# LouisRouss/DiffuLab

Hardware: AMD Instinct MI355X
Metric: train images/sec/node (DiT-S/2 flow-matching, 256x256 latents) (higher is better)
Workload: dtype bf16

## Files before the change

diffulab_amd/csrc/block.hip:

```cpp
#include <stdlib.h>

#include "common.h"

static thread_local hipEvent_t g_blk_event = nullptr;
static int fork_to_side(hipStream_t main, hipStream_t side) {
  if (main == side) return 0;
  if (!g_blk_event && hipEventCreateWithFlags(&g_blk_event, hipEventDisableTiming) != hipSuccess) return -1;
  if (hipEventRecord(g_blk_event, main) != hipSuccess) return -1;
  return hipStreamWaitEvent(side, g_blk_event, 0) == hipSuccess ? 0 : -1;
}

extern "C" int dl_stream_wait_stream(dl_stream_t waiter, dl_stream_t waited) {
  if (fork_to_side((hipStream_t)waited, (hipStream_t)waiter) != 0) {
    dl_set_error("dl_stream_wait_stream: %s", hipGetErrorString(hipGetLastError()));
    return DL_ERR_LAUNCH;
  }
  return DL_OK;
}
extern "C" int dl_memset_zero(void* p, int64_t bytes, dl_stream_t stream) {
  DL_CHECK_ARG(p && bytes >= 0, "dl_memset_zero: bad args");
  if (bytes && hipMemsetAsync(p, 0, (size_t)bytes, (hipStream_t)stream) != hipSuccess) {
    dl_set_error("dl_memset_zero: %s", hipGetErrorString(hipGetLastError()));
    return DL_ERR_LAUNCH;
  }
// ... 77 lines not shown
  if (rc == DL_ERR_UNSUPPORTED) {
    DL_CHECK_ARG(P(U), "dl_dit_block_fwd: this shape has no fused MLP-up kernel and needs the U buffer");
    RUN(dl_gemm_nt(P(XM2), D, P(W_UP), b->ldw_d, P(U), 2 * F, M, 2 * F, D, nullptr, DL_ACT_NONE, DL_BF16, nullptr, nullptr, 0, nullptr, 0, 1,
                   stream));
    RUN(dl_swiglu_fwd(P(U), P(H), M, F, stream));
  } else if (rc != DL_OK) {
    return rc;
  }
  RUN(dl_gemm_nt(P(H), F, P(W_DOWN), b->ldw_f, P(T2), D, M, D, F, nullptr, DL_ACT_NONE, DL_BF16, nullptr, nullptr, 0, nullptr, 0, 1, stream));
  return DL_OK;
}

extern "C" int dl_dit_block_bwd(const dl_dit_block_t* b, dl_stream_t main_, dl_stream_t side_, int side_wgs) {
  DL_CHECK_ARG(b, "dl_dit_block_bwd: null block");
  hipStream_t main = (hipStream_t)main_, side = (hipStream_t)side_;
  const DlWgCapScope cap_scope(b->max_workgroups);
  const int64_t B = b->B, N = b->N, D = b->D, H = b->H, F = b->F, M = B * N, dh = D / H;
  const float sm = 0.125f;
  dl_wgrad_t wg[4];
  int nwg = 0;
  bool grouped = P(TN_SLAB) != nullptr && ((D % 384 == 0 && F % 192 == 0) || (D % 256 == 0 && F % 256 == 0)) && M % 32 == 0 && M >= 2048;
  auto wgrad = [&](const void* dy, int64_t ldy, const void* x, int64_t ldx, void* g, int64_t Mo, int64_t No) -> int {
    if (grouped) {
      wg[nwg++] = dl_wgrad_t{dy, ldy, x, ldx, (float*)g, Mo, No};
      return DL_OK;
    }
    if (fork_to_side(main, side)) return DL_ERR_LAUNCH;
    return dl_gemm_tn_ex(dy, ldy, x, ldx, (float*)g, No, Mo, No, M, side_wgs, side);
  };
  auto fold = [&](void* partial, void* g) -> int {
    if (fork_to_side(main, side)) return DL_ERR_LAUNCH;
    return dl_reduce_rows_f32((float*)partial, (float*)g, B, 2 * D, 1, side);
  };
  RUN(wgrad(P(DT2), D, P(H), F, P(G_DOWN), D, F));
  if (P(U)) {
    RUN(dl_gemm_nt(P(DT2), D, P(WT_DOWN), b->ldwt_d, P(DH), F, M, F, D, nullptr, DL_ACT_NONE, DL_BF16, nullptr, nullptr, 0, nullptr, 0, 1, main));
    RUN(dl_swiglu_bwd(P(DH), P(U), P(DU), M, F, main));
  } else {
    RUN(dl_mlp_dswiglu_recompute(P(XM2), D, P(W_UP_PERM), b->ldw_d, P(DT2), D, P(WT_DOWN), b->ldwt_d, P(DU), 2 * F, M, F, D, D, main));
  }
  RUN(wgrad(P(DU), 2 * F, P(XM2), D, P(G_UP), 2 * F, D));
  const bool rows = (b->row_gemms & 1) != 0, fold_here = (b->row_gemms & 4) == 0;
  if (rows) {
    RUN(dl_ln_modulate_gemm_bwd(P(DU), 2 * F, P(WT_UP), b->ldwt_f2, M, 2 * F, P(X1), (const float*)P(LN2_W), (const float*)P(LN2_B),
                                P(SCALE2), b->ld_mod, N, (const float*)P(MEAN2), (const float*)P(RSTD2), P(DX_IN), P(DX_MID),
                                (float*)P(DSCALE2), (float*)P(DSHIFT2), b->ld_dmod, (float*)P(DWB2), P(T1), P(GATE1), b->ld_mod, P(DT1),
                                (float*)P(DGATE1), D, main));
  } else {
    RUN(dl_gemm_nt(P(DU), 2 * F, P(WT_UP), b->ldwt_f2, P(DXM), D, M, D, 2 * F, nullptr, DL_ACT_NONE, DL_BF16, nullptr, nullptr, 0, nullptr,
                   0, 1, main));
    RUN(dl_ln_modulate_bwd(P(DXM), P(X1), (const float*)P(LN2_W), (const float*)P(LN2_B), P(SCALE2), b->ld_mod, N,
                           (const float*)P(MEAN2), (const float*)P(RSTD2), P(DX_IN), P(DX_MID), (float*)P(DSCALE2), (float*)P(DSHIFT2),
                           b->ld_dmod, (float*)P(DWB2), P(T1), P(GATE1), b->ld_mod, P(DT1), (float*)P(DGATE1), M, D, main));
  }
  if (fold_here) RUN(fold(P(DWB2), P(G_LN2)));
  RUN(wgrad(P(DT1), D, P(A), D, P(G_PROJ), D, D));
  RUN(dl_gemm_nt(P(DT1), D, P(WT_PROJ), b->ldwt_d, P(DA), D, M, D, D, nullptr, DL_ACT_NONE, DL_BF16, nullptr, nullptr, 0, nullptr, 0, 1, main));
  const bool v_in_place = P(V) == nullptr;
  if (v_in_place && P(QK_PARTIALS) && D <= 512) {
    RUN(dl_attn_bwd_tok(P(Q), P(K), P(QKV), P(A), P(DA), (const float*)P(LSE), P(DQKV), B, H, N, dh, sm, main));
    RUN(dl_qk_norm_rope_bwd_inplace(P(QKV), (const float*)P(QN_SCALE), (const float*)P(KN_SCALE), (const float*)P(ROPE_COS),
                                    (const float*)P(ROPE_SIN), (const float*)P(RRMS), P(DQKV), (float*)P(G_QK_SCALE),
                                    (float*)P(QK_PARTIALS), B, N, H, dh, b->rot, nullptr, main));
  } else {
    if (v_in_place)
      RUN(dl_attn_bwd_sv(P(Q), P(K), (const char*)P(QKV) + 2 * D * 2, N * 3 * D, dh, 3 * D, P(A), P(DA), (const float*)P(LSE), P(DQ), P(DK),
// ... 31 lines not shown
```

diffulab_amd/csrc/block_fused.hip:

```cpp
#include <stdlib.h>

#include "common.h"
#include "attention_body.h"
#include "gemm_rows_body.h"
#include "gemm_stationary_body.h"

#define CH_THREADS 512
#define CH_NKS 6

struct ChainRowGemm {
  const bf16_t* A;
  int64_t lda;
  const bf16_t* W;
  int64_t ldw;
  int K;
  RowEpi ep;
};
struct ChainAttn {
  const bf16_t* qkv;
  bf16_t* out;
  float* lse;
  int H;
  float scale;
  QkNorm qn;
};
struct ChainArgs {
  int B;
  StArgs qkv;
  ChainAttn attn;
  ChainRowGemm proj;
  StArgs up;
  ChainRowGemm down;
};

constexpr int ch_max(int a, int b) { return a > b ? a : b; }
constexpr int ch_lds_bytes() { return ch_max(ch_max(st_lds_bytes<CH_NKS>(), 2 * RK_STAGE), attn_pipe_lds_bytes(RK_BN)); }

static __device__ __forceinline__ void ch_phase_sync() {
  asm volatile("s_waitcnt vmcnt(0) lgkmcnt(0)" ::: "memory");
  __builtin_amdgcn_fence(__ATOMIC_RELEASE, "workgroup");
  __syncthreads();
  __builtin_amdgcn_fence(__ATOMIC_ACQUIRE, "workgroup");
}

static __device__ __forceinline__ const ChainArgs* ch_args() {
  auto p = __builtin_amdgcn_kernarg_segment_ptr();
  asm volatile("" : "+s"(p));
  return (const ChainArgs*)p;
}
static __device__ __forceinline__ int ch_tid() {
  int t = threadIdx.x;
  asm volatile("" : "+v"(t));
  return t;
}
static __device__ __forceinline__ void ch_row_gemm(const ChainRowGemm* gp, char* smem, int sample) {
  const ChainRowGemm g = *gp;
  rk_gemm_body<RK_LNF>(g.A, g.lda, g.W, g.ldw, RK_BN, g.K, g.ep, smem, ch_tid(), sample, 0, 1);
}
template <int EPI>
static __device__ __forceinline__ void ch_st_gemm(const StArgs* ap, char* smem, int sample) {
  const StArgs a = *ap;
  st_gemm_body<CH_NKS, EPI>(a, smem, ch_tid(), sample, 0, 1);
}
static __device__ __forceinline__ void ch_attention(const ChainAttn* ap, char* smem, int sample) {
  const ChainAttn a = *ap;
  attn_qkn_pipe_body(a.qkv, a.out, a.lse, a.H, a.scale, a.qn, smem, ch_tid(), sample * a.H, 1, a.H);
}

__global__ __launch_bounds__(CH_THREADS, 2) void dit_block_fwd_chain_k(ChainArgs a) {
  extern __shared__ __attribute__((aligned(16))) char smem[];
  for (int s = blockIdx.x; s < a.B; s += gridDim.x) {
    ch_st_gemm<1>(&ch_args()->qkv, smem, s);
    ch_phase_sync();
    ch_attention(&ch_args()->attn, smem, s);
    ch_phase_sync();
    ch_row_gemm(&ch_args()->proj, smem, s);
    ch_phase_sync();
    ch_st_gemm<0>(&ch_args()->up, smem, s);
    ch_phase_sync();
    ch_row_gemm(&ch_args()->down, smem, s);
    ch_phase_sync();
  }
}

#define P(k) (b->p[DL_BLK_##k])
#define CH_ALIGNED16(p) ((((uintptr_t)(p)) & 15) == 0)

static void ch_row_epi(RowEpi& ep, const void* resid, const void* gate, int64_t ld_gate, const void* ln_w, const void* ln_b,
                       const void* scale, const void* shift, int64_t ld_mod, float eps, void* t_out, void* x_out, void* xm_out,
                       void* mean, void* rstd) {
// ... 59 lines not shown
                     (const float*)P(ROPE_SIN), (bf16_t*)(train ? P(Q) : nullptr), (bf16_t*)(train ? P(K) : nullptr),
                     (float*)(train ? P(RRMS) : nullptr), 1.0f / (float)D, 1e-6f, (int)b->rot, (int)(3 * D)};
  a.proj.A = (const bf16_t*)P(A);
  a.proj.lda = D;
  a.proj.W = (const bf16_t*)P(W_PROJ);
  a.proj.ldw = b->ldw_d;
  a.proj.K = (int)D;
  ch_row_epi(a.proj.ep, P(X_IN), P(GATE1), b->ld_mod, P(LN2_W), P(LN2_B), P(SCALE2), P(SHIFT2), b->ld_mod, b->eps, P(T1), P(X1), P(XM2),
             P(MEAN2), P(RSTD2));
  a.up = StArgs{(const bf16_t*)P(XM2), D, (const bf16_t*)P(W_UP_PERM), b->ldw_d, (bf16_t*)u, 2 * F, (bf16_t*)P(H), F, (int)F, nullptr, 0,
                (int)(B * N), (int)(2 * F)};
  a.down.A = (const bf16_t*)P(H);
  a.down.lda = F;
  a.down.W = (const bf16_t*)P(W_DOWN);
  a.down.ldw = b->ldw_f;
  a.down.K = (int)F;
  ch_row_epi(a.down.ep, P(X1), P(GATE2), b->ld_mod, P(NEXT_LN_W), P(NEXT_LN_B), P(NEXT_SCALE), P(NEXT_SHIFT), b->ld_mod, b->next_eps,
             P(T2), P(NEXT_X), P(NEXT_XM), P(NEXT_MEAN), P(NEXT_RSTD));

  constexpr int LDS = ch_lds_bytes();
  static_assert(LDS <= 160 * 1024, "the chain kernel's LDS is the largest phase's");
  static DevOnce once;
  const int n_cu = dev_cus(once, [] {
    (void)hipFuncSetAttribute((const void*)dit_block_fwd_chain_k, hipFuncAttributeMaxDynamicSharedMemorySize, LDS);
  });
  const DlWgCapScope cap_scope(b->max_workgroups);
  const int budget = dl_wg_budget(n_cu);
  int grid = (int)(B < budget ? B : budget);
  if (b->max_workgroups > 0 && b->max_workgroups < grid) grid = b->max_workgroups;
  hipLaunchKernelGGL(dit_block_fwd_chain_k, grid, CH_THREADS, LDS, (hipStream_t)stream, a);
  DL_LAUNCH_CHECK();
  return DL_OK;
}
```

diffulab_amd/csrc/gemm_stationary_body.h:

```cpp
#ifndef DIFFULAB_GEMM_STATIONARY_BODY_H
#define DIFFULAB_GEMM_STATIONARY_BODY_H

#include <type_traits>

#include "common.h"

#define ST_THREADS 512
#define ST_PANEL 256
#define ST_ROWS 64

typedef __attribute__((address_space(3))) void st_lds_void_t;
typedef const __attribute__((address_space(1))) void st_glb_void_t;

struct StArgs {
  const bf16_t* X;
  int64_t ldx;
  const bf16_t* W;
  int64_t ldw;
  bf16_t* C;
  int64_t ldc;
  bf16_t* H;
  int64_t ldh;
  int F;
  float* ssq;
// ... 96 lines not shown
          auto sh = __builtin_amdgcn_permlane32_swap(__float_as_uint(hv[e]), __float_as_uint(hv[4 + e]), false, false);
          v1[e] = __uint_as_float(s1[0]);
          v1[4 + e] = __uint_as_float(s1[1]);
          v3[e] = __uint_as_float(s3[0]);
          v3[4 + e] = __uint_as_float(s3[1]);
          h8[e] = __uint_as_float(sh[0]);
          h8[4 + e] = __uint_as_float(sh[1]);
        }
#pragma unroll
        for (int e = 0; e < 16; ++e) c[e] = 0.f;
        if (a.C) {
          *(u32x4_t*)(a.C + (int64_t)m * a.ldc + u0) = pack8(v1);
          *(u32x4_t*)(a.C + (int64_t)m * a.ldc + a.F + u0) = pack8(v3);
        }
        *(u32x4_t*)(a.H + (int64_t)m * a.ldh + u0) = pack8(h8);
      }
    } else {
#pragma unroll
      for (int j = 0; j < 2; ++j)
#pragma unroll
        for (int gp = 0; gp < 2; ++gp) {
          f32x16_t& c = acc[2 * HALF + j];
          float v[8];
#pragma unroll
          for (int e = 0; e < 4; ++e) {
            auto sw2 = __builtin_amdgcn_permlane32_swap(__float_as_uint(c[8 * gp + e]), __float_as_uint(c[8 * gp + 4 + e]), false, false);
            v[e] = __uint_as_float(sw2[0]);
            v[4 + e] = __uint_as_float(sw2[1]);
            c[8 * gp + e] = 0.f;
            c[8 * gp + 4 + e] = 0.f;
          }
          const u32x4_t pk = pack8(v);
          *(u32x4_t*)(a.C + (int64_t)m * a.ldc + n_base + j * 32 + 16 * gp + 8 * hi) = pk;
          float r[8];
          unpack8(pk, r);
#pragma unroll
          for (int e = 0; e < 8; ++e) ss += r[e] * r[e];
        }
      if (st % 6 == 2) {
        ss_lo = xor32_sum(ss);
        ss = 0.f;
      }
      if ((st + 1) % 6 == 0 || st + 1 == S) {
        if (st / 6 < a.ssq_tiles) {
          const float t = ss_lo + xor32_sum(ss);
          if (hi == 0) a.ssq[(int64_t)m * a.ssq_tiles + st / 6] = t;
        }
        ss = 0.f;
        ss_lo = 0.f;
      }
    }
  };

  int it = 0;
  auto stage = [&](auto half_tag, int st) {
    constexpr int HALF = decltype(half_tag)::value;
    constexpr int YOUNG = (NST - 2) * NKS;
    if (it + NST - 2 < total) {
      if (st < 2) st_wait_vmcnt<YOUNG>();
      else if (EPI == 1) st_wait_vmcnt<YOUNG + 4>();
      else if (a.C) st_wait_vmcnt<YOUNG + 6>();
      else st_wait_vmcnt<YOUNG + 2>();
    } else {
      st_wait_vmcnt<0>();
    }
    __builtin_amdgcn_s_barrier();
    if (NST < 3 && s_it < total) stage_next();
    if (upper && st > 0) epilogue(std::integral_constant<int, 1 - HALF>{}, st - 1);
    const unsigned sw = smem_lds + (it % NST) * STAGE + rd_base;
    bf16x8_t wq[PD + 1];
    auto rd = [&](int s) {
      const int f = s >> 1;
      const unsigned ad = sw + (((f & 7) << 5) ^ rd_x);
      bf16x8_t& v = wq[s % (PD + 1)];
      switch ((f >> 3) * 2 + (s & 1)) {
        case 0: st_lds_read<0>(v, ad); break;
        case 1: st_lds_read<32 * PITCH>(v, ad); break;
        case 2: st_lds_read<256>(v, ad); break;
        case 3: st_lds_read<32 * PITCH + 256>(v, ad); break;
        case 4: st_lds_read<512>(v, ad); break;
        case 5: st_lds_read<32 * PITCH + 512>(v, ad); break;
        case 6: st_lds_read<768>(v, ad); break;
        default: st_lds_read<32 * PITCH + 768>(v, ad); break;
      }
    };
#pragma unroll
    for (int s = 0; s < PD; ++s) rd(s);
#pragma unroll
    for (int s = 0; s < 2 * NF; ++s) {
      __builtin_amdgcn_sched_barrier(0);
      if (s + PD < 2 * NF) rd(s + PD);
      st_lds_landed_n(2 * NF - 1 - s < PD ? 2 * NF - 1 - s : PD, wq[s % (PD + 1)]);
      acc[2 * HALF + (s & 1)] =
// ... 29 lines not shown
```

diffulab_amd/engine.py:

```python

from __future__ import annotations

import functools
import math
from dataclasses import dataclass, field

import torch
from torch import Tensor

from . import ops, tuning


_PARAM_EPOCH = 0


def bump_param_epoch() -> None:
    global _PARAM_EPOCH
    _PARAM_EPOCH += 1


def _must(ok: bool) -> None:
    if not ok:
        raise RuntimeError("a HIP kernel declined a shape the engine had selected it for")

# ... 584 lines not shown
        blk.ldwt_3d = sh[pre + "attention.qkv.weight|t"].stride(0)
        blk.rot, blk.eps = sum(d.rope_axes_dim), 1e-5
        blk.max_workgroups = self._main_wgs()
        prev = None
        if i > 0:
            ap = w["layers"][(i - 1) if train else 0]
            prev = (ap["x1"], ap["t2"], mrow((i - 1) * 6 * D + 5 * D))
        blk.set(x_in=xin, pend_x=prev[0] if prev else None, pend_t=prev[1] if prev else None, pend_gate=prev[2] if prev else None,
                scale1=mrow(mo), shift1=mrow(mo + D), gate1=mrow(mo + 2 * D), scale2=mrow(mo + 3 * D), shift2=mrow(mo + 4 * D),
                gate2=mrow(mo + 5 * D),
                ln1_w=self.P(pre + "norm_1.weight"), ln1_b=self.P(pre + "norm_1.bias"), ln2_w=self.P(pre + "norm_2.weight"),
                ln2_b=self.P(pre + "norm_2.bias"), qn_scale=self.P(pre + "attention.qk_norm.query_norm.scale"),
                kn_scale=self.P(pre + "attention.qk_norm.key_norm.scale"),
                w_qkv=sh[pre + "attention.qkv.weight|f"], w_proj=sh[pre + "attention.proj_out.weight|f"],
                w_up=sh[pre + "mlp_input.0.weight|f"], w_up_perm=sh[pre + "mlp_input.0.weight|g"], w_down=sh[pre + "mlp_input.2.weight|f"],
                wt_qkv=sh[pre + "attention.qkv.weight|t"], wt_proj=sh[pre + "attention.proj_out.weight|t"],
                wt_up=sh[pre + "mlp_input.0.weight|t"], wt_down=sh[pre + "mlp_input.2.weight|t"], rope_cos=cos, rope_sin=sin,
                xm1=a["xm1"], mean1=a["mean1"], rstd1=a["rstd1"], qkv=a["qkv"], q=a["q"], k=a["k"], v=a["v"], rrms=a["rrms"], a=a["a"],
                lse=a["lse"], t1=a["t1"], x1=a["x1"], xm2=a["xm2"], mean2=a["mean2"], rstd2=a["rstd2"], u=a["u"], h=a["h"], t2=a["t2"],
                ssq=w["ssq_all"][i] if "ssq_all" in w else None)
        rows = self._row_gemms(M, N)
        blk.row_gemms = 0
        if rows:
            if i + 1 < L:
                nx, mn, nxt = w["layers"][(i + 1) if train else 0], (i + 1) * 6 * D, f"layers.{i + 1}."
                lnw, lnb, blk.next_eps = self.P(nxt + "norm_1.weight"), self.P(nxt + "norm_1.bias"), 1e-5
                xm_n, mu_n, rs_n = nx["xm1"], nx["mean1"], nx["rstd1"]
            else:
                mn, lnw, lnb, blk.next_eps = L * 6 * D, None, None, 1e-6
                xm_n, mu_n, rs_n = w["xf"], w["meanf"], w["rstdf"]
            blk.set(next_ln_w=lnw, next_ln_b=lnb, next_scale=mrow(mn), next_shift=mrow(mn + D),
                    next_x=xs[i + 1] if train else xs[(i + 1) & 1], next_xm=xm_n, next_mean=mu_n, next_rstd=rs_n)
            blk.row_gemms = (1 | (2 if tuning.on("DL_ROW_GEMM_QK") else 0) | (4 if self.reducer is None else 0)
                             | (8 if tuning.on("DL_BLOCK_CHAIN") else 0))
        if train and self.grads is not None:
            g, dmod = w["wg"][i], w["dmod32"]
            blk.ld_dmod = dmod.stride(0)
            drow = lambda off: dmod.data_ptr() + 4 * off
            pg = None
            if i > 0:
                mp = (i - 1) * 6 * D
                pg = (w["layers"][i - 1]["t2"], mrow(mp + 5 * D), w["wg"][i - 1]["dt2"], drow(mp + 5 * D))
            blk.set(dt2=g["dt2"], dx_in=w["dxa"], dx_mid=w["dxb"], dx_out=w["dxa"], dh=w["dh"], du=g["du"], dxm=w["dxm"], dt1=g["dt1"],
                    da=w["da"], dq=w["dq"], dk=w["dk"], dv=w["dv"], dqkv=g["dqkv"], dfeat=None,
                    dscale1=drow(mo), dshift1=drow(mo + D), dgate1=drow(mo + 2 * D), dscale2=drow(mo + 3 * D), dshift2=drow(mo + 4 * D),
                    dwb1=w["dwb"][2 * i], dwb2=w["dwb"][2 * i + 1],
                    prev_t2=pg[0] if pg else None, prev_gate2=pg[1] if pg else None, prev_dt2=pg[2] if pg else None,
                    prev_dgate2=pg[3] if pg else None,
                    g_qkv=self.G(pre + "attention.qkv.weight"), g_proj=self.G(pre + "attention.proj_out.weight"),
                    g_up=self.G(pre + "mlp_input.0.weight"), g_down=self.G(pre + "mlp_input.2.weight"),
                    g_ln1=self.G(pre + "norm_1.weight"), g_ln2=self.G(pre + "norm_2.weight"),
                    g_qk_scale=self.G(pre + "attention.qk_norm.query_norm.scale"), tn_slab=w.get("tn_slab"),
                    qk_partials=w.get("qk_part"))
            blk.tn_slab_floats = w["tn_slab"].numel() if "tn_slab" in w else 0
        self._blk_cache[key] = blk
        return blk

    def forward(self, x: Tensor, t: Tensor, y_eff: Tensor | None, train: bool = True, refresh: bool = True) -> Tensor:
        d = self.d
        B, C, H, W = x.shape
        assert C == d.input_channels and x.dtype == torch.float32 and x.is_cuda
        self._alloc(B, H, W, train)
        if refresh:
            self.refresh_shadows(force=train)
        w, sh = self.ws, self.sh
        _, _, _, gh, gw, N, M, _, _ = self.geo
        D, L = d.inner_dim, d.depth
# ... 614 lines not shown
```

diffulab_amd/ops.py:

```python

from __future__ import annotations

import ctypes
import os

import torch
from torch import Tensor

from ._lib import lib
from . import tuning

BF16, F32 = 0, 1
ACT_NONE, ACT_SILU, ACT_GELU = 0, 1, 2
LOSS_FLOW, LOSS_EPS = 0, 1
MEAN_TYPES = {"epsilon": 0, "xstart": 1, "xprev": 2, "v": 3}
VAR_MODES = {"learned": 0, "learned_range": 1}
VAR_FIXED = -1
PATCH_CPP, PATCH_PPC = 0, 1


_raw_stream = getattr(torch._C, "_cuda_getCurrentRawStream", None)


def _s() -> int:
# ... 768 lines not shown
          float(scale), _s())


ATTN_MAX_TOKENS = 32768
_INT32_ELEMS = 2 ** 31


def check_row_extent(rows: int, width: int, what: str) -> None:
    if rows * width >= _INT32_ELEMS:
        raise NotImplementedError(f"{what}: {rows} token rows x {width} columns = {rows * width} elements exceed the 2^31 elements the "
                                  "bf16 regime's kernels index; use a smaller batch")


def attn_needs_padding(N: int) -> bool:
    return N % 64 != 0 or (N > 256 and N % 256 != 0)


def v_in_place(N: int) -> bool:
    return N <= 256 and N % 64 == 0 and tuning.on("DL_ATTN_V_IN_PLACE")


def dit_block_fwd(blk, train: bool) -> None:
    _call("dl_dit_block_fwd", ctypes.addressof(blk), int(train), _s())


def dit_block_fwd_chain(blk, train: bool) -> bool:
    return _maybe("dl_dit_block_fwd_chain", ctypes.addressof(blk), int(train), _s())


def dit_block_bwd(blk, main_stream: int, side_stream: int, side_wgs: int) -> None:
    _call("dl_dit_block_bwd", ctypes.addressof(blk), main_stream, side_stream, int(side_wgs))


def attn_fwd_qkv(q, k, qkv, out, lse, B, H, N, dh, scale):
    D = H * dh
    _call("dl_attn_fwd_sv", _p(q), _p(k), qkv.data_ptr() + 2 * D * 2, N * 3 * D, dh, 3 * D, _p(out), _p(lse), B, H, N, dh,
          float(scale), _s())


def gemm_nt_ssq(a, w_sh, out, ssq, stationary: bool = False, max_workgroups: int = 0) -> bool:
    args = (_p(a), a.stride(0), _p(w_sh), w_sh.stride(0), _p(out), out.stride(0), a.shape[0], w_sh.shape[0], a.shape[1], _p(ssq), ssq.shape[1])
    if stationary and _maybe("dl_gemm_nt_ssq_stationary", *args, int(max_workgroups), _s()):
        return True
    return _maybe("dl_gemm_nt_ssq", *args, _s())


def attn_fwd_qkn(qkv, ssq, scale_q, scale_k, cos, sin, q, k, rrms, out, lse, B, H, N, dh, rot, scale, eps=1e-6):
    _call("dl_attn_fwd_qkn", _p(qkv), _p(ssq), _p(scale_q), _p(scale_k), _p(cos), _p(sin), float(eps), rot, _p(q), _p(k), _p(rrms), _p(out),
          _p(lse), B, H, N, dh, float(scale), _s())


def attn_bwd_qkv(q, k, qkv, out, dout, lse, dq, dk, dqkv, B, H, N, dh, scale):
    D = H * dh
    _call("dl_attn_bwd_sv", _p(q), _p(k), qkv.data_ptr() + 2 * D * 2, N * 3 * D, dh, 3 * D, _p(out), _p(dout), _p(lse), _p(dq),
          _p(dk), dqkv.data_ptr() + 2 * D * 2, N * 3 * D, dh, 3 * D, B, H, N, dh, float(scale), _s())


def attn_bwd_tok(q, k, qkv, out, dout, lse, dqkv, B, H, N, dh, scale):
    _call("dl_attn_bwd_tok", _p(q), _p(k), _p(qkv), _p(out), _p(dout), _p(lse), _p(dqkv), B, H, N, dh, float(scale), _s())


def qk_inplace_ok(ws: dict, B: int, tokens: int) -> bool:
    return ws.get("qk_part") is not None and v_in_place(tokens) and B * tokens >= 32768


def qk_norm_rope_bwd_inplace(qkv, scale_q, scale_k, cos, sin, rrms, dqkv, dscale, partials, B, N, H, dh, rot, pos=None) -> bool:
# ... 756 lines not shown
```

diffulab_amd/tuning.py:

```python

from __future__ import annotations

import os

SWITCHES: dict[str, tuple[str, str]] = {
    "DL_NATIVE_BLOCK": ("1", "DiT blocks issued by the C ABI's block drivers (dl_dit_block_fwd / _bwd) instead of one Python call per kernel"),
    "DL_ROW_GEMM": ("1", "LayerNorm-modulate forward / backward as epilogues of the row-complete 256x384 GEMMs (D = 384, 256 tokens per sample)"),
    "DL_ROW_GEMM_QK": ("0", "QK-norm + RoPE as the epilogue of the qkv GEMM (measured slower than the separate row kernel)"),
    "DL_QKN_ON_LOAD": ("1", "QK-RMSNorm statistics leave with the qkv GEMM (dl_gemm_nt_ssq) and norm + RoPE are applied as the attention "
                       "forward stages q and k (dl_attn_fwd_qkn): no qk_norm_rope_fwd pass (row-complete path, <= 256 tokens)"),
    "DL_BLOCK_CHAIN": ("1", "block forward of the row-complete path as one per-sample chain launch (dl_dit_block_fwd_chain; native block "
                       "driver, 256 tokens per sample, QK-norm on load)"),
    "DL_MLP_RECOMPUTE": ("1", "SwiGLU backward recomputes the MLP-up pre-activations instead of storing them in the forward"),
    "DL_ATTN_V_IN_PLACE": ("1", "attention reads V / writes dV inside the token-major qkv rows (N <= 256)"),
    "DL_QK_INPLACE": ("1", "attention backward writes dQ / dK token-major and the QK-norm backward runs in place on the dqkv rows"),
    "DL_WGRAD_GROUP": ("1", "the four weight gradients of a block as one atomics-free launch (dl_gemm_tn_group)"),
    "DL_WGRAD_INLINE": ("0", "grouped weight gradients on the main stream instead of the side stream"),
    "DL_WGRAD_SERIAL": ("0", "per-problem weight gradients on the main stream (engines without the grouped form)"),
    "DL_SIDE_WGS": ("", "workgroup cap of the side-stream weight gradients (default: 256 grouped, 128 per-problem)"),
    "DL_SIDE_CU_MASK": ("", "CU mask of the side stream (dl_stream_create_masked): 'i4' = every 4th CU, 'b128' = the first 128"),
    "DL_SIDE_LOW_PRIORITY": ("0", "DiT engines: the side stream of the weight gradients is created with the device's lowest stream priority "
                             "(measured +-0: DiT-S/2 20.83 / 20.80 vs 20.73 / 20.77 ms; SPRINT joint 28.77 / 28.58 vs 28.79 / 28.62; DDT 38.93 / 38.97 vs "
                             "39.01 / 39.00; joint MMDiT 49.14 / 49.13 vs 49.24 / 49.31; REPA 11.71 / 11.68 vs 11.76 / 11.73)"),
    "DL_UNET_SIDE_LOW_PRIORITY": ("1", "UNet: the same (the dispatcher serves the main chain's workgroups first: 26.42 / 26.50 vs 26.66 / 26.64 ms)"),
    "DL_JOIN_LAST": ("1", "single GPU: the side stream is joined after the conditioning backward instead of before it"),
    "DL_DP_RESERVE_CUS": ("0", "data parallel: CUs left to the communication library's workgroups (persistent main-chain grids shrink by it; "
                          "measured a loss at the headline shape, whose tile counts are whole multiples of 256: DESIGN.md section 5)"),
    "DL_MAIN_WGS": ("", "workgroup budget of the persistent main-chain kernels (experiments; default: all CUs, or CUs - reserve with a reducer)"),
    "DL_DP_EARLY_MOD": ("1", "data parallel: each block's adaLN rows are reduced as the block finishes"),
    "DL_HIPGRAPH": ("1", "samplers replay the denoiser forward as a captured hipGraph"),
    "DL_CFG_PAIR": ("1", "guided sampler steps run the conditional and the label-dropped forward as ONE forward over [x ; x] "
                    "(class-conditional MMDiT / DDT / UNetModel: same values per row, the weights stream once)"),
    "DL_LAUNCH_PLAN": ("0", "UNet (bf16 regime): a training forward / backward is recorded on its second run for a shape and re-issued as a "
                       "flat list of C calls afterwards (ops.LaunchPlan: the engine's Python costs the host ~24 us per launch, 716 "
                       "launches per step).  Measured (profiles/r06_e_*): the step at B = 64 is NOT host-bound -- its main queue is busy "
                       "19.2 of 20.3 ms and `host_issue` is the full launch queue pushing back -- so the plan changes nothing there "
                       "(20.03 vs 20.11 ms); it pays where the host is the slower side (under a profiler's per-launch overhead: 20.3 vs "
                       "22.7 ms), hence opt-in"),
    "DL_UNET_SIDE": ("1", "UNet weight gradients on a side stream"),
    "DL_UNET_NT_PAIR": ("1", "UNet AttentionBlock: the q and kv projections (and their data gradients) as one launch of the 128 x 128 GEMM "
                        "kernel where both are small (dl_gemm_nt_pair: 64 + 128 tiles on 256 CUs at the 4 x 4 level); bit-identical"),
    "DL_UNET_XATTN_HIP": ("1", "UNet TransformerBlock (context conditioning): the cross-attention core as dl_attn_cross_* (bf16 operands, f32 "
                          "softmax; MFMA with the keys streamed in 64-key tiles where dh % 64 == 0, VALU otherwise) where Nq <= 64, L <= 512, "
                          "dh % 8 == 0; 0 = the f32 copies + batched dl_f32_gemm + masked softmax fallback"),
    "DL_UNET_SPLITK": ("1", "split-K convolutions at the UNet's low-resolution levels (partial images + fixed-order fold: -7 % per step)"),
# ... 28 lines not shown
```

include/diffulab_hip.h:

```cpp
#ifndef DIFFULAB_HIP_H
#define DIFFULAB_HIP_H

#include <stdint.h>

#ifdef __cplusplus
extern "C" {
#endif

#define DL_API __attribute__((visibility("default")))

typedef void* dl_stream_t;

enum { DL_OK = 0, DL_ERR_INVALID = -1, DL_ERR_LAUNCH = -2, DL_ERR_UNSUPPORTED = -3 };
enum { DL_BF16 = 0, DL_F32 = 1 };
enum { DL_ACT_NONE = 0, DL_ACT_SILU = 1, DL_ACT_GELU = 2 };
enum { DL_LOSS_FLOW = 0, DL_LOSS_EPS = 1 };
enum { DL_MEAN_EPSILON = 0, DL_MEAN_XSTART = 1, DL_MEAN_XPREV = 2, DL_MEAN_V = 3 };
enum { DL_VAR_LEARNED = 0, DL_VAR_LEARNED_RANGE = 1 };
enum { DL_VAR_FIXED = -1 };
enum { DL_PATCH_CPP = 0, DL_PATCH_PPC = 1 };

DL_API int dl_version(void);
DL_API const char* dl_last_error(void);
DL_API int dl_device_info(int device, int* cu_count, int* lds_bytes_per_cu, int64_t* hbm_bytes, char* arch,
// ... 525 lines not shown
  DL_BLK_DT2,
  DL_BLK_DX_IN,
  DL_BLK_DX_MID,
  DL_BLK_DX_OUT,
  DL_BLK_DH, DL_BLK_DU, DL_BLK_DXM, DL_BLK_DT1, DL_BLK_DA, DL_BLK_DQ, DL_BLK_DK, DL_BLK_DV, DL_BLK_DQKV, DL_BLK_DFEAT ,
  DL_BLK_DSCALE1, DL_BLK_DSHIFT1, DL_BLK_DGATE1, DL_BLK_DSCALE2, DL_BLK_DSHIFT2,
  DL_BLK_DWB1, DL_BLK_DWB2,
  DL_BLK_PREV_T2, DL_BLK_PREV_GATE2, DL_BLK_PREV_DT2, DL_BLK_PREV_DGATE2,
  DL_BLK_G_QKV, DL_BLK_G_PROJ, DL_BLK_G_UP, DL_BLK_G_DOWN, DL_BLK_G_LN1, DL_BLK_G_LN2, DL_BLK_G_QK_SCALE,
  DL_BLK_NEXT_LN_W, DL_BLK_NEXT_LN_B, DL_BLK_NEXT_SCALE, DL_BLK_NEXT_SHIFT,
  DL_BLK_NEXT_X,
  DL_BLK_NEXT_XM, DL_BLK_NEXT_MEAN, DL_BLK_NEXT_RSTD,
  DL_BLK_TN_SLAB,
  DL_BLK_QK_PARTIALS,
  DL_BLK_SSQ,
  DL_BLK_NPTR
};
typedef struct dl_dit_block_t {
  void* p[96];
  int64_t B, N, D, H, F;
  int64_t ld_mod, ld_dmod;
  int64_t ldw_d, ldw_f;
  int64_t ldwt_d, ldwt_f2, ldwt_3d;
  int64_t rot;
  float eps;
  float next_eps;
  int32_t row_gemms;
  int64_t tn_slab_floats;
  int32_t max_workgroups;
} dl_dit_block_t;
DL_API int dl_dit_block_fwd(const dl_dit_block_t* blk, int train, dl_stream_t stream);
DL_API int dl_dit_block_fwd_chain(const dl_dit_block_t* blk, int train, dl_stream_t stream);
DL_API int dl_dit_block_bwd(const dl_dit_block_t* blk, dl_stream_t main_stream, dl_stream_t side_stream, int side_workgroups);

#ifdef __cplusplus
}
#endif
#endif
```

Measured before the change: 12890.

## Fuse sample-local DiT block backward phases into per-sample chain kernels

```diff
diff --git a/diffulab_amd/csrc/block.hip b/diffulab_amd/csrc/block.hip
--- a/diffulab_amd/csrc/block.hip
+++ b/diffulab_amd/csrc/block.hip
@@ -133,6 +133,23 @@
     if (fork_to_side(main, side)) return DL_ERR_LAUNCH;
     return dl_reduce_rows_f32((float*)partial, (float*)g, B, 2 * D, 1, side);
   };
+  if ((b->row_gemms & 16) && (b->row_gemms & 1) && grouped) {
+    const int rc = dl_dit_block_bwd_chain(b, main_);
+    if (rc == DL_OK) {
+      RUN(wgrad(P(DT2), D, P(H), F, P(G_DOWN), D, F));
+      RUN(wgrad(P(DU), 2 * F, P(XM2), D, P(G_UP), 2 * F, D));
+      RUN(wgrad(P(DT1), D, P(A), D, P(G_PROJ), D, D));
+      RUN(wgrad(P(DQKV), 3 * D, P(XM1), D, P(G_QKV), 3 * D, D));
+      if (fork_to_side(main, side)) return DL_ERR_LAUNCH;
+      RUN(dl_gemm_tn_group(wg, nwg, M, (float*)P(TN_SLAB), b->tn_slab_floats, side_wgs, side));
+      if ((b->row_gemms & 4) == 0) {
+        RUN(fold(P(DWB2), P(G_LN2)));
+        RUN(fold(P(DWB1), P(G_LN1)));
+      }
+      return DL_OK;
+    }
+    if (rc != DL_ERR_UNSUPPORTED) return rc;
+  }
   RUN(wgrad(P(DT2), D, P(H), F, P(G_DOWN), D, F));
   if (P(U)) {
     RUN(dl_gemm_nt(P(DT2), D, P(WT_DOWN), b->ldwt_d, P(DH), F, M, F, D, nullptr, DL_ACT_NONE, DL_BF16, nullptr, nullptr, 0, nullptr, 0, 1, main));
diff --git a/diffulab_amd/csrc/block_fused.hip b/diffulab_amd/csrc/block_fused.hip
--- a/diffulab_amd/csrc/block_fused.hip
+++ b/diffulab_amd/csrc/block_fused.hip
@@ -4,6 +4,7 @@
 #include "attention_body.h"
 #include "gemm_rows_body.h"
 #include "gemm_stationary_body.h"
+#include "qk_norm_bwd_body.h"
 
 #define CH_THREADS 512
 #define CH_NKS 6
@@ -43,19 +44,21 @@
   __builtin_amdgcn_fence(__ATOMIC_ACQUIRE, "workgroup");
 }
 
-static __device__ __forceinline__ const ChainArgs* ch_args() {
+template <class Args = ChainArgs>
+static __device__ __forceinline__ const Args* ch_args() {
   auto p = __builtin_amdgcn_kernarg_segment_ptr();
   asm volatile("" : "+s"(p));
-  return (const ChainArgs*)p;
+  return (const Args*)p;
 }
 static __device__ __forceinline__ int ch_tid() {
   int t = threadIdx.x;
   asm volatile("" : "+v"(t));
   return t;
 }
+template <int MODE = RK_LNF>
 static __device__ __forceinline__ void ch_row_gemm(const ChainRowGemm* gp, char* smem, int sample) {
   const ChainRowGemm g = *gp;
-  rk_gemm_body<RK_LNF>(g.A, g.lda, g.W, g.ldw, RK_BN, g.K, g.ep, smem, ch_tid(), sample, 0, 1);
+  rk_gemm_body<MODE>(g.A, g.lda, g.W, g.ldw, RK_BN, g.K, g.ep, smem, ch_tid(), sample, 0, 1);
 }
 template <int EPI>
 static __device__ __forceinline__ void ch_st_gemm(const StArgs* ap, char* smem, int sample) {
@@ -181,3 +184,209 @@
   DL_LAUNCH_CHECK();
   return DL_OK;
 }
+
+int dl_fold_rows_launch(const float* partial, float* out, int G, int n, hipStream_t stream);
+
+struct ChainQkb {
+  const bf16_t* qkv;
+  const float* sq;
+  const float* sk;
+  const float* cs;
+  const float* sn;
+  const float* rrms;
+  bf16_t* dqkv;
+  float* partials;
+  int H, rot;
+};
+struct BwdChainArgs {
+  int B;
+  ChainRowGemm ln2;
+  StArgs proj;
+  ChainQkb qkb;
+  ChainRowGemm ln1;
+};
+#define CHB_A 1
+#define CHB_B 2
+
+static __device__ __forceinline__ void ch_qk_bwd(const ChainQkb* ap, char* smem, int sample, bool first) {
+  const ChainQkb a = *ap;
+  const int tid = ch_tid();
+  const int lane = tid & 63, wave = tid >> 6;
+  const QkbLane c = qkb_lane(lane, a.H, 64, a.rot);
+  const int D = c.D;
+  float wq[8], wk[8], aq[8], ak[8];
+#pragma unroll
+  for (int e = 0; e < 8; ++e) {
+    wq[e] = c.on ? a.sq[c.col + e] : 0.f;
+    wk[e] = c.on ? a.sk[c.col + e] : 0.f;
+    aq[e] = ak[e] = 0.f;
+  }
+  const int64_t r0 = (int64_t)sample * RK_BM;
+  QkbRow n0, n1;
+  auto fetch = [&](QkbRow& n, int t) { qkb_fetch(n, c, a.qkv, a.dqkv, a.rrms, a.cs, a.sn, r0 + t, t); };
+  auto row = [&](QkbRow& n, int t, bool more) {
+    float xq[8], xk[8], gq[8], gk[8];
+    unpack8(n.xq, xq);
+    unpack8(n.xk, xk);
+    unpack8(n.gq, gq);
+    unpack8(n.gk, gk);
+    const f32x4_t cc = n.cc, ss = n.ss;
+    const float rq = n.rq, rk = n.rk;
+    if (more) fetch(n, t + 16);
+    qkb_row(xq, xk, gq, gk, cc, ss, rq, rk, c, wq, wk, aq, ak, a.dqkv, r0 + t);
+  };
+  fetch(n0, wave);
+  fetch(n1, wave + 8);
+  for (int t = wave; t < RK_BM; t += 16) {
+    row(n0, t, t + 16 < RK_BM);
+    row(n1, t + 8, t + 16 < RK_BM);
+  }
+  float* red = (float*)smem;
+  if (c.on) {
+#pragma unroll
+    for (int e = 0; e < 8; ++e) {
+      red[(size_t)wave * 2 * D + c.col + e] = aq[e];
+      red[(size_t)wave * 2 * D + D + c.col + e] = ak[e];
+    }
+  }
+  __syncthreads();
+  for (int i = tid; i < 2 * D; i += CH_THREADS) {
+    float s[8];
+#pragma unroll
+    for (int w = 0; w < 8; ++w) s[w] = red[(size_t)w * 2 * D + i];
+    const float t = ((s[0] + s[1]) + (s[2] + s[3])) + ((s[4] + s[5]) + (s[6] + s[7]));
+    float* p = a.partials + (size_t)blockIdx.x * 2 * D + i;
+    *p = first ? t : *p + t;
+  }
+}
+
+template <int PHASES>
+__global__ __launch_bounds__(CH_THREADS, 2) void dit_block_bwd_chain_k(BwdChainArgs a) {
+  extern __shared__ __attribute__((aligned(16))) char smem[];
+  bool first = true;
+  for (int s = blockIdx.x; s < a.B; s += gridDim.x) {
+    if constexpr (PHASES & CHB_A) {
+      ch_row_gemm<RK_LNB>(&ch_args<BwdChainArgs>()->ln2, smem, s);
+      ch_phase_sync();
+      {
+        const StArgs p = ch_args<BwdChainArgs>()->proj;
+        st_gemm_body<CH_NKS, 2>(p, smem, ch_tid(), s, 0, 1);
+      }
+      ch_phase_sync();
+    }
+    if constexpr (PHASES & CHB_B) {
+      ch_qk_bwd(&ch_args<BwdChainArgs>()->qkb, smem, s, first);
+      first = false;
+      ch_phase_sync();
+      ch_row_gemm<RK_LNB>(&ch_args<BwdChainArgs>()->ln1, smem, s);
+      ch_phase_sync();
+    }
+  }
+}
+
+static void ch_row_epi_bwd(RowEpi& ep, const void* x, const void* ln_w, const void* ln_b, const void* scale, int64_t ld_mod,
+                           const void* mean, const void* rstd, const void* dres, void* dx, void* dscale, void* dshift, int64_t ld_dmod,
+                           void* dwb, const void* gate_t, const void* gate, int64_t ld_gate, void* dt, void* dgate) {
+  ep.x = (const bf16_t*)x;
+  ep.ln_w = (const float*)ln_w;
+  ep.ln_b = (const float*)ln_b;
+  ep.scale = (const bf16_t*)scale;
+  ep.ld_mod = ld_mod;
+  ep.mean_i = (const float*)mean;
+  ep.rstd_i = (const float*)rstd;
+  ep.dres = (const bf16_t*)dres;
+  ep.dx = (bf16_t*)dx;
+  ep.dscale = (float*)dscale;
+  ep.dshift = (float*)dshift;
+  ep.ld_dmod = ld_dmod;
+  ep.dwb = (float*)dwb;
+  ep.gt = (const bf16_t*)gate_t;
+  ep.gate = (const bf16_t*)gate;
+  ep.ld_gate = ld_gate;
+  ep.gdt = (bf16_t*)dt;
+  ep.dgate = (float*)dgate;
+}
+
+template <int PHASES>
+static int chb_launch(const BwdChainArgs& a, int grid, hipStream_t stream) {
+  constexpr int LDS = ch_lds_bytes();
+  static DevOnce once;
+  (void)dev_cus(once, [] {
+    (void)hipFuncSetAttribute((const void*)dit_block_bwd_chain_k<PHASES>, hipFuncAttributeMaxDynamicSharedMemorySize, LDS);
+  });
+  hipLaunchKernelGGL(dit_block_bwd_chain_k<PHASES>, grid, CH_THREADS, LDS, stream, a);
+  DL_LAUNCH_CHECK();
+  return DL_OK;
+}
+
+extern "C" int dl_dit_block_bwd_chain(const dl_dit_block_t* b, dl_stream_t main) {
+  DL_CHECK_ARG(b, "dl_dit_block_bwd_chain: null block");
+  const int64_t B = b->B, N = b->N, D = b->D, H = b->H, F = b->F, M = B * N;
+  DL_CHECK_ARG(B > 0 && N > 0 && D > 0 && H > 0 && F > 0, "dl_dit_block_bwd_chain: bad dims");
+  if (!(b->row_gemms & 1) || P(V) || !P(QK_PARTIALS) || !P(TN_SLAB) || P(U) || P(DFEAT) || N != RK_BM || D != RK_BN || D != H * 64 ||
+      H % 2 || F % 128 || F % 192 || M < 2048 || B * (F / 128) < 64 || M >= (1ll << 31) || F >= (1ll << 28)) {
+    dl_set_error("dl_dit_block_bwd_chain: needs row_gemms bit 0, V in place, QK_PARTIALS, TN_SLAB, no U, no DFEAT, N == 256, D == 384, "
+                 "head_dim == 64, an even head count, F %% 128 == 0, F %% 192 == 0, 8 samples and 64 MLP tiles (B=%lld N=%lld D=%lld H=%lld F=%lld)",
+                 (long long)B, (long long)N, (long long)D, (long long)H, (long long)F);
+    return DL_ERR_UNSUPPORTED;
+  }
+  DL_CHECK_ARG(P(XM2) && P(W_UP_PERM) && P(DT2) && P(WT_DOWN) && P(DU) && P(WT_UP) && P(X1) && P(SCALE2) && P(MEAN2) && P(RSTD2) &&
+                   P(DX_MID) && P(DSCALE2) && P(DSHIFT2) && P(T1) && P(GATE1) && P(DT1) && P(DGATE1) && P(WT_PROJ) && P(DA),
+               "dl_dit_block_bwd_chain: null operand (MLP branch / projection)");
+  DL_CHECK_ARG(P(Q) && P(K) && P(QKV) && P(A) && P(LSE) && P(DQKV) && P(QN_SCALE) && P(KN_SCALE) && P(RRMS) && P(G_QK_SCALE) &&
+                   b->rot >= 0 && b->rot % 8 == 0 && b->rot <= 64 && (b->rot == 0 || (P(ROPE_COS) && P(ROPE_SIN))) && P(WT_QKV) &&
+                   P(X_IN) && P(SCALE1) && P(MEAN1) && P(RSTD1) && P(DX_OUT) && P(DSCALE1) && P(DSHIFT1),
+               "dl_dit_block_bwd_chain: null operand (attention branch / LN1), or rot not a multiple of 8 up to 64");
+  DL_CHECK_ARG((P(LN1_W) == nullptr) == (P(LN1_B) == nullptr) && (P(LN2_W) == nullptr) == (P(LN2_B) == nullptr),
+               "dl_dit_block_bwd_chain: LayerNorm w and b must both be given or both NULL");
+  DL_CHECK_ARG(!P(PREV_T2) || (P(PREV_GATE2) && P(PREV_DT2) && P(PREV_DGATE2)),
+               "dl_dit_block_bwd_chain: the previous block's gate backward needs PREV_T2, PREV_GATE2, PREV_DT2 and PREV_DGATE2");
+  DL_CHECK_ARG(b->ldw_d % 8 == 0 && b->ldw_d >= D && b->ldwt_d % 8 == 0 && b->ldwt_d >= D && b->ldwt_f2 % 8 == 0 && b->ldwt_f2 >= 2 * F &&
+                   b->ldwt_3d % 8 == 0 && b->ldwt_3d >= 3 * D && b->ld_mod % 8 == 0 && b->ldw_d < (1ll << 20) && b->ldwt_d < (1ll << 20) &&
+                   b->ldwt_f2 < (1ll << 20) && b->ldwt_3d < (1ll << 20),
+               "dl_dit_block_bwd_chain: leading dimensions");
+  DL_CHECK_ARG(CH_ALIGNED16(P(XM2)) && CH_ALIGNED16(P(W_UP_PERM)) && CH_ALIGNED16(P(DT2)) && CH_ALIGNED16(P(WT_DOWN)) && CH_ALIGNED16(P(DU)) &&
+                   CH_ALIGNED16(P(WT_UP)) && CH_ALIGNED16(P(X1)) && CH_ALIGNED16(P(SCALE2)) && CH_ALIGNED16(P(DX_IN)) &&
+                   CH_ALIGNED16(P(DX_MID)) && CH_ALIGNED16(P(T1)) && CH_ALIGNED16(P(GATE1)) && CH_ALIGNED16(P(DT1)) && CH_ALIGNED16(P(LN2_W)) &&
+                   CH_ALIGNED16(P(WT_PROJ)) && CH_ALIGNED16(P(DA)) && CH_ALIGNED16(P(QKV)) && CH_ALIGNED16(P(DQKV)) &&
+                   CH_ALIGNED16(P(ROPE_COS)) && CH_ALIGNED16(P(ROPE_SIN)) && CH_ALIGNED16(P(WT_QKV)) && CH_ALIGNED16(P(X_IN)) &&
+                   CH_ALIGNED16(P(SCALE1)) && CH_ALIGNED16(P(DX_OUT)) && CH_ALIGNED16(P(PREV_T2)) && CH_ALIGNED16(P(PREV_GATE2)) &&
+                   CH_ALIGNED16(P(PREV_DT2)) && CH_ALIGNED16(P(LN1_W)),
+               "dl_dit_block_bwd_chain: 16-byte alignment");
+
+  BwdChainArgs a{};
+  a.B = (int)B;
+  a.ln2.A = (const bf16_t*)P(DU);
+  a.ln2.lda = 2 * F;
+  a.ln2.W = (const bf16_t*)P(WT_UP);
+  a.ln2.ldw = b->ldwt_f2;
+  a.ln2.K = (int)(2 * F);
+  ch_row_epi_bwd(a.ln2.ep, P(X1), P(LN2_W), P(LN2_B), P(SCALE2), b->ld_mod, P(MEAN2), P(RSTD2), P(DX_IN), P(DX_MID), P(DSCALE2), P(DSHIFT2),
+                 b->ld_dmod, P(DWB2), P(T1), P(GATE1), b->ld_mod, P(DT1), P(DGATE1));
+  a.proj = StArgs{(const bf16_t*)P(DT1), D, (const bf16_t*)P(WT_PROJ), b->ldwt_d, (bf16_t*)P(DA), D, nullptr, 0, 0, nullptr, 0, (int)M, (int)D};
+  a.qkb = ChainQkb{(const bf16_t*)P(QKV), (const float*)P(QN_SCALE), (const float*)P(KN_SCALE), (const float*)P(ROPE_COS),
+                   (const float*)P(ROPE_SIN), (const float*)P(RRMS), (bf16_t*)P(DQKV), (float*)P(QK_PARTIALS), (int)H, (int)b->rot};
+  a.ln1.A = (const bf16_t*)P(DQKV);
+  a.ln1.lda = 3 * D;
+  a.ln1.W = (const bf16_t*)P(WT_QKV);
+  a.ln1.ldw = b->ldwt_3d;
+  a.ln1.K = (int)(3 * D);
+  ch_row_epi_bwd(a.ln1.ep, P(X_IN), P(LN1_W), P(LN1_B), P(SCALE1), b->ld_mod, P(MEAN1), P(RSTD1), P(DX_MID), P(DX_OUT), P(DSCALE1), P(DSHIFT1),
+                 b->ld_dmod, P(DWB1), P(PREV_T2), P(PREV_GATE2), b->ld_mod, P(PREV_DT2), P(PREV_DGATE2));
+
+  static_assert(ch_lds_bytes() <= 160 * 1024, "the chain kernel's LDS is the largest phase's");
+  static DevOnce once;
+  const int n_cu = dev_cus(once, [] {});
+  const DlWgCapScope cap_scope(b->max_workgroups);
+  const int budget = dl_wg_budget(n_cu);
+  int grid = (int)(B < budget ? B : budget);
+  if (b->max_workgroups > 0 && b->max_workgroups < grid) grid = b->max_workgroups;
+  if (grid > 768) grid = 768;
+  hipStream_t stream = (hipStream_t)main;
+  int rc = dl_mlp_dswiglu_recompute(P(XM2), D, P(W_UP_PERM), b->ldw_d, P(DT2), D, P(WT_DOWN), b->ldwt_d, P(DU), 2 * F, M, F, D, D, main);
+  if (rc != DL_OK) return rc == DL_ERR_UNSUPPORTED ? DL_ERR_INVALID : rc;
+  if ((rc = chb_launch<CHB_A>(a, grid, stream)) != DL_OK) return rc;
+  if ((rc = dl_attn_bwd_tok(P(Q), P(K), P(QKV), P(A), P(DA), (const float*)P(LSE), P(DQKV), B, H, N, 64, 0.125f, main)) != DL_OK) return rc;
+  if ((rc = chb_launch<CHB_B>(a, grid, stream)) != DL_OK) return rc;
+  return dl_fold_rows_launch((const float*)P(QK_PARTIALS), (float*)P(G_QK_SCALE), grid, (int)(2 * D), stream);
+}
diff --git a/diffulab_amd/csrc/gemm_stationary_body.h b/diffulab_amd/csrc/gemm_stationary_body.h
--- a/diffulab_amd/csrc/gemm_stationary_body.h
+++ b/diffulab_amd/csrc/gemm_stationary_body.h
@@ -152,11 +152,14 @@
           }
           const u32x4_t pk = pack8(v);
           *(u32x4_t*)(a.C + (int64_t)m * a.ldc + n_base + j * 32 + 16 * gp + 8 * hi) = pk;
-          float r[8];
-          unpack8(pk, r);
-#pragma unroll
-          for (int e = 0; e < 8; ++e) ss += r[e] * r[e];
-        }
+          if constexpr (EPI == 1) {
+            float r[8];
+            unpack8(pk, r);
+#pragma unroll
+            for (int e = 0; e < 8; ++e) ss += r[e] * r[e];
+          }
+        }
+      if constexpr (EPI != 1) return;
       if (st % 6 == 2) {
         ss_lo = xor32_sum(ss);
         ss = 0.f;
@@ -178,7 +181,7 @@
     constexpr int YOUNG = (NST - 2) * NKS;
     if (it + NST - 2 < total) {
       if (st < 2) st_wait_vmcnt<YOUNG>();
-      else if (EPI == 1) st_wait_vmcnt<YOUNG + 4>();
+      else if (EPI != 0) st_wait_vmcnt<YOUNG + 4>();
       else if (a.C) st_wait_vmcnt<YOUNG + 6>();
       else st_wait_vmcnt<YOUNG + 2>();
     } else {
diff --git a/diffulab_amd/csrc/qk_norm_bwd_body.h b/diffulab_amd/csrc/qk_norm_bwd_body.h
--- /dev/null
+++ b/diffulab_amd/csrc/qk_norm_bwd_body.h
@@ -0,0 +1,84 @@
+#ifndef DIFFULAB_QK_NORM_BWD_BODY_H
+#define DIFFULAB_QK_NORM_BWD_BODY_H
+
+#include "common.h"
+
+struct QkbLane {
+  int D, col, d0, rot;
+  bool on, rope;
+  float invD;
+};
+static __device__ __forceinline__ QkbLane qkb_lane(int lane, int H, int dh, int rot) {
+  QkbLane c;
+  c.D = H * dh;
+  c.on = lane < (c.D >> 3);
+  c.invD = 1.0f / (float)c.D;
+  c.col = lane * 8;
+  const int hh = c.on ? c.col / dh : 0;
+  c.d0 = c.col - hh * dh;
+  c.rot = rot;
+  c.rope = c.on && c.d0 < rot;
+  return c;
+}
+
+struct QkbRow {
+  u32x4_t xq = {0, 0, 0, 0}, xk = {0, 0, 0, 0}, gq = {0, 0, 0, 0}, gk = {0, 0, 0, 0};
+  f32x4_t cc = {0.f, 0.f, 0.f, 0.f}, ss = {0.f, 0.f, 0.f, 0.f};
+  float rq = 0.f, rk = 0.f;
+};
+static __device__ __forceinline__ void qkb_fetch(QkbRow& n, const QkbLane& c, const bf16_t* __restrict__ qkv, const bf16_t* dqkv,
+                                                 const float* __restrict__ rrms, const float* __restrict__ cs,
+                                                 const float* __restrict__ sn, int64_t r, int nt) {
+  const bf16_t* p = qkv + r * 3 * c.D + c.col;
+  const bf16_t* g = dqkv + r * 3 * c.D + c.col;
+  if (c.on) {
+    n.xq = *(const u32x4_t*)p;
+    n.xk = *(const u32x4_t*)(p + c.D);
+    n.gq = *(const u32x4_t*)g;
+    n.gk = *(const u32x4_t*)(g + c.D);
+  }
+  n.rq = rrms[r * 2];
+  n.rk = rrms[r * 2 + 1];
+  if (c.rope) {
+    n.cc = *(const f32x4_t*)(cs + (int64_t)nt * (c.rot >> 1) + (c.d0 >> 1));
+    n.ss = *(const f32x4_t*)(sn + (int64_t)nt * (c.rot >> 1) + (c.d0 >> 1));
+  }
+}
+static __device__ __forceinline__ void qkb_row(float (&xq)[8], float (&xk)[8], float (&gq)[8], float (&gk)[8], const f32x4_t cc,
+                                               const f32x4_t ss, const float rq, const float rk, const QkbLane& c, const float (&wq)[8],
+                                               const float (&wk)[8], float (&aq)[8], float (&ak)[8], bf16_t* dqkv, int64_t row) {
+#pragma clang fp contract(off)
+  if (c.rope) {
+#pragma unroll
+    for (int i = 0; i < 4; ++i) {
+      const float qa = gq[2 * i], qb = gq[2 * i + 1], ka = gk[2 * i], kb = gk[2 * i + 1];
+      gq[2 * i] = qa * cc[i] + qb * ss[i];
+      gq[2 * i + 1] = __builtin_fmaf(qb, cc[i], -(qa * ss[i]));
+      gk[2 * i] = ka * cc[i] + kb * ss[i];
+      gk[2 * i + 1] = __builtin_fmaf(kb, cc[i], -(ka * ss[i]));
+    }
+  }
+  float s1 = 0.f, s2 = 0.f;
+#pragma unroll
+  for (int e = 0; e < 8; ++e) {
+    aq[e] = __builtin_fmaf(gq[e] * xq[e], rq, aq[e]);
+    ak[e] = __builtin_fmaf(gk[e] * xk[e], rk, ak[e]);
+    gq[e] *= wq[e];
+    gk[e] *= wk[e];
+    s1 += gq[e] * xq[e];
+    s2 += gk[e] * xk[e];
+  }
+  const float mq = wave_sum(s1) * c.invD * rq * rq * rq, mk = wave_sum(s2) * c.invD * rk * rk * rk;
+#pragma unroll
+  for (int e = 0; e < 8; ++e) {
+    gq[e] = __builtin_fmaf(rq, gq[e], -(xq[e] * mq));
+    gk[e] = __builtin_fmaf(rk, gk[e], -(xk[e] * mk));
+  }
+  if (c.on) {
+    bf16_t* o = dqkv + row * 3 * c.D + c.col;
+    *(u32x4_t*)o = pack8(gq);
+    *(u32x4_t*)(o + c.D) = pack8(gk);
+  }
+}
+
+#endif
diff --git a/diffulab_amd/engine.py b/diffulab_amd/engine.py
--- a/diffulab_amd/engine.py
+++ b/diffulab_amd/engine.py
@@ -640,7 +640,7 @@
             blk.set(next_ln_w=lnw, next_ln_b=lnb, next_scale=mrow(mn), next_shift=mrow(mn + D),
                     next_x=xs[i + 1] if train else xs[(i + 1) & 1], next_xm=xm_n, next_mean=mu_n, next_rstd=rs_n)
             blk.row_gemms = (1 | (2 if tuning.on("DL_ROW_GEMM_QK") else 0) | (4 if self.reducer is None else 0)
-                             | (8 if tuning.on("DL_BLOCK_CHAIN") else 0))
+                             | (8 if tuning.on("DL_BLOCK_CHAIN") else 0) | (16 if tuning.on("DL_BLOCK_CHAIN_BWD") else 0))
         if train and self.grads is not None:
             g, dmod = w["wg"][i], w["dmod32"]
             blk.ld_dmod = dmod.stride(0)
diff --git a/diffulab_amd/ops.py b/diffulab_amd/ops.py
--- a/diffulab_amd/ops.py
+++ b/diffulab_amd/ops.py
@@ -824,6 +824,10 @@
     _call("dl_dit_block_bwd", ctypes.addressof(blk), main_stream, side_stream, int(side_wgs))
 
 
+def dit_block_bwd_chain(blk, main_stream: int) -> bool:
+    return _maybe("dl_dit_block_bwd_chain", ctypes.addressof(blk), main_stream)
+
+
 def attn_fwd_qkv(q, k, qkv, out, lse, B, H, N, dh, scale):
     D = H * dh
     _call("dl_attn_fwd_sv", _p(q), _p(k), qkv.data_ptr() + 2 * D * 2, N * 3 * D, dh, 3 * D, _p(out), _p(lse), B, H, N, dh,
diff --git a/diffulab_amd/tuning.py b/diffulab_amd/tuning.py
--- a/diffulab_amd/tuning.py
+++ b/diffulab_amd/tuning.py
@@ -11,6 +11,8 @@
                        "forward stages q and k (dl_attn_fwd_qkn): no qk_norm_rope_fwd pass (row-complete path, <= 256 tokens)"),
     "DL_BLOCK_CHAIN": ("1", "block forward of the row-complete path as one per-sample chain launch (dl_dit_block_fwd_chain; native block "
                        "driver, 256 tokens per sample, QK-norm on load)"),
+    "DL_BLOCK_CHAIN_BWD": ("1", "block backward: the sample-local phases of the main chain as per-sample chain launches "
+                           "(dl_dit_block_bwd_chain; native block driver, 256 tokens per sample, grouped weight gradients)"),
     "DL_MLP_RECOMPUTE": ("1", "SwiGLU backward recomputes the MLP-up pre-activations instead of storing them in the forward"),
     "DL_ATTN_V_IN_PLACE": ("1", "attention reads V / writes dV inside the token-major qkv rows (N <= 256)"),
     "DL_QK_INPLACE": ("1", "attention backward writes dQ / dK token-major and the QK-norm backward runs in place on the dqkv rows"),
diff --git a/include/diffulab_hip.h b/include/diffulab_hip.h
--- a/include/diffulab_hip.h
+++ b/include/diffulab_hip.h
@@ -581,6 +581,7 @@
 DL_API int dl_dit_block_fwd(const dl_dit_block_t* blk, int train, dl_stream_t stream);
 DL_API int dl_dit_block_fwd_chain(const dl_dit_block_t* blk, int train, dl_stream_t stream);
 DL_API int dl_dit_block_bwd(const dl_dit_block_t* blk, dl_stream_t main_stream, dl_stream_t side_stream, int side_workgroups);
+DL_API int dl_dit_block_bwd_chain(const dl_dit_block_t* blk, dl_stream_t main_stream);
 
 #ifdef __cplusplus
 }
```

Result: no change. 13010, median of 6 (+0.9%).
